# muzishen/RCDMs

Measured on AMD Instinct MI355X. Metric: story-frames/sec (stage-2 UNet, 50-step DDIM, 512^2), higher is better.
Workload: dtype f16; 1 GPU; PororoSV stage-2, 512x512, 50-step DDIM, CFG 2.0, batch=1 story x 5 frames per GPU, ctx 85x768, random-init 1276.9M-param UNet3D; stories_per_gpu=1, latent=64, ddim_steps=50, parallelism=story-replicas x1

## Files before the change

include/rcdm.h:

```cpp
#ifndef RCDM_H
#define RCDM_H

#include <stddef.h>
#include <stdint.h>

#ifdef __cplusplus
extern "C" {
#endif

#define RCDM_VERSION 0x000300

#define RCDM_OK 0
#define RCDM_EINVAL (-1)
#define RCDM_ESHAPE (-2)
#define RCDM_ELAUNCH (-3)
#define RCDM_EWORKSPACE (-4)
#define RCDM_ECOMM (-5)

#define RCDM_EPI_BIAS 1
#define RCDM_EPI_ROWVEC 2
#define RCDM_EPI_RESIDUAL 4
#define RCDM_EPI_GELU 16
#define RCDM_EPI_GEGLU 8
#define RCDM_EPI_QUICK_GELU 32
// ... 124 lines not shown
int rcdm_pack_conv3x3_wino(const float* w, int32_t c_out, int32_t c_in, void* dst, void* stream);
int rcdm_upsample_taps_gather(const void* P, int32_t ldp, int32_t n_img, int32_t h, int32_t w, int32_t c_out, const float* bias,
                              void* out, int32_t ldc, void* stream);
int rcdm_conv_taps_gather(const void* P, int32_t ldp, int32_t n_img, int32_t h, int32_t w, int32_t c_out, int32_t upsample,
                          const float* bias, void* out, int32_t ldc, void* stream);
int rcdm_set_wino_slab_f16(int32_t on);
int rcdm_conv3x3_wino(const rcdm_conv3x3_desc* d, const rcdm_groupnorm_desc* gn, const float* gn_stat,
                      const float* gn_gamma, const float* gn_beta, const void* in, const void* in2, const void* U,
                      const void* W2, const float* bias, const float* rowvec, const void* residual, void* out,
                      void* workspace, size_t workspace_bytes, const rcdm_groupnorm_desc* gn_out, float* gn_out_partial,
                      void* stream);

typedef struct {
  int32_t M, C, ldx, ldy;
  float eps;
  int32_t rows_per_frame, frames;
} rcdm_layernorm_desc;

int rcdm_layernorm(const rcdm_layernorm_desc* d, const void* x, const float* gamma,
                   const float* beta, const float* pe, void* y, void* stream);

#define RCDM_ATTN_WIDE_RANGE 1
typedef struct {
  int32_t batch, heads, Lq, Lk, d;
  int32_t ldq, ldk, ldv, ldo;
  float scale;
  int32_t flags;
} rcdm_attn_desc;

int rcdm_flash_attn(const rcdm_attn_desc* d, const void* Q, const void* K, const void* V, void* out,
                    void* stream);
int rcdm_flash_attn_masked(const rcdm_attn_desc* d, const void* Q, const void* K, const void* V,
                           const unsigned char* key_valid, int32_t causal, void* out, void* stream);

size_t rcdm_xattn_image_bytes(int32_t batch, int32_t heads, int32_t d);
int rcdm_xattn_pack_kv(const void* K, const void* V, int32_t batch, int32_t Lk, int32_t heads, int32_t d, int32_t ldk,
                       int32_t ldv, void* image, void* stream);
int rcdm_xattn(const rcdm_attn_desc* d, const void* Q, const void* image, void* out, void* stream);

typedef struct {
  int32_t samples, frames, pixels, heads, d;
  int32_t ldqkv, ldo;
  float scale;
} rcdm_temporal_attn_desc;

int rcdm_temporal_attn(const rcdm_temporal_attn_desc* d, const void* qkv, void* out, void* stream);

typedef struct {
  int32_t M, C;
  int32_t ldx, ldo;
  float eps;
} rcdm_ff_desc;
size_t rcdm_ff_stream_bytes(int32_t C);
int rcdm_ff_fused_supported(int32_t C);
int rcdm_pack_ff_stream(const float* w1, const float* b1, const float* w2, int32_t C, void* wstream, float* b1_packed,
                        void* stream);
int rcdm_ff_fused(const rcdm_ff_desc* d, const void* x, const float* ln_gamma, const float* ln_beta, const void* wstream,
                  const float* b1_packed, const float* b2, void* out, void* stream);

typedef struct {
  int32_t M, C;
  int32_t lda, ldr, ldt, ldo;
  int32_t tail;
  int32_t rows_per_frame, frames;
  float eps;
  int32_t gn_groups, gn_rows;
// ... 324 lines not shown
```

rcdms_amd/csrc/attn.hip:

```cpp
#include <stdlib.h>
#include "common.h"
#include "attn_wide.h"

long long* g_attn_trace = nullptr;

namespace {

constexpr int KT = 64;

struct AttnArgs {
  const f16* Q;
  const f16* K;
  const f16* V;
  f16* O;
  int batch, heads, Lq, Lk, d, dch;
  int ldq, ldk, ldv, ldo;
  float c;
  const unsigned char* kvalid;
  int causal;
  int plain_order;
  int wide;
  long long* trace;
};

// ... 10 lines not shown
  return r;
}

constexpr float MSUB_THR = 6.0f;

template <int DS, int QF, bool PIPE, bool MASKED, int NW, int MD = 0>
__global__ __launch_bounds__(NW * 64, (MASKED && DS >= 5) ? 1 : 2) void flash_attn_kernel(const AttnArgs p) {
  constexpr bool MSUB = MD > 0;
  static_assert(!MSUB || (PIPE && !MASKED && MD < 16 * DS), "MSUB: pipelined, unmasked kernel with a spare QK^T column only");
  constexpr int DF = (DS + 1) / 2;
  constexpr int KP = 16 * DS + 8;
  constexpr int NT = NW * 64;
  constexpr int NSLOT = (KT * 2 * DS + NT - 1) / NT;
  constexpr int BQ = NW * 32 * QF;
  constexpr int VR = v_row_halfs(DF);
  constexpr int SK = KT * KP, SV = KT * VR;
  extern __shared__ __attribute__((aligned(16))) char smem[];
  f16* sK = (f16*)smem;
  f16* sV = sK + 2 * SK;

  const int t = threadIdx.x, lane = t & 63, wave = t >> 6;
  const int lr = lane & 31, hi = lane >> 5;
  const int nqb = (p.Lq + BQ - 1) / BQ;
  int item;
  {
    const int total = nqb * p.heads * p.batch, lin = blockIdx.x;
    const int xcd = lin & 7, q = total >> 3, r = total & 7;
    item = (xcd < r ? xcd * (q + 1) : r * (q + 1) + (xcd - r) * q) + (lin >> 3);
    if (p.plain_order) item = lin;
  }
  const int qb = item % nqb, bh = item / nqb;
  const int h = bh % p.heads, b = bh / p.heads;
  const int q0 = qb * BQ + wave * 32 * QF + lr;
  const bool ones_row = (DS & 1) ? true : p.d < 32 * DF;

  for (int i = t; i < (2 * SK + 2 * SV) / 8; i += NT) ((uint4*)smem)[i] = make_uint4(0, 0, 0, 0);
  __syncthreads();
  if (ones_row && t < 2 * KT) sV[(t >> 6) * SV + (t & 63) * VR + p.d] = (f16)1.0f;
  if (MSUB && t < 2 * KT) sK[(t >> 6) * SK + (t & 63) * KP + p.d] = (f16)1.0f;
  constexpr int sd_frag = MD >> 4, sd_hi = (MD >> 3) & 1, sd_e = MD & 7;

  f16x8 qf[QF][DS];
#pragma unroll
  for (int j = 0; j < QF; ++j)
#pragma unroll
    for (int s = 0; s < DS; ++s) {
      const int dc = s * 16 + hi * 8;
      Pack16 v;
      v.u = make_uint4(0, 0, 0, 0);
      if (q0 + 32 * j < p.Lq && dc < p.d)
        v.u = *(const uint4*)(p.Q + ((size_t)b * p.Lq + q0 + 32 * j) * p.ldq + h * p.d + dc);
      if (MSUB) {
#pragma unroll
        for (int e = 0; e < 8; ++e) v.e[e] = (f16)((float)v.e[e] * p.c);
      }
      qf[j][s] = v.h;
    }
  float m_sub[QF], m_issue[QF];
#pragma unroll
  for (int j = 0; j < QF; ++j) m_sub[j] = m_issue[j] = 0.f;

  f32x16 oacc[QF][DF];
  float m_run[QF], l_run[QF];
#pragma unroll
  for (int j = 0; j < QF; ++j) {
    m_run[j] = -INFINITY;
// ... 220 lines not shown
    }

    RCDM_ATTN_STAMP(tr_sm);
#pragma unroll
    for (int f = 0; f < DF; ++f)
#pragma unroll
      for (int st = 0; st < 4; ++st) {
        const f16* vp = sV + par * SV + v_rd + (16 * st) * VR + 32 * f;
        union { s16x4 h[2]; f16x8 v; } vf;
        vf.h[0] = lds_read_tr16(vp);
        vf.h[1] = lds_read_tr16(vp + 8 * VR);
#pragma unroll
        for (int j = 0; j < QF; ++j) oacc[j][f] = __builtin_amdgcn_mfma_f32_32x32x16_f16(vf.v, pf[j][st], oacc[j][f], 0, 0, 0);
        if constexpr (DS == 10) __builtin_amdgcn_sched_barrier(0);
      }
    RCDM_ATTN_STAMP(tr_pv);
  };

  if constexpr (PIPE) {
    for (int kt = 0; kt < ntiles; kt += 2) {
      step(kt, s_even, s_odd);
      if (kt + 1 < ntiles) step(kt + 1, s_odd, s_even);
    }
  } else {
    for (int kt = 0; kt < ntiles; ++kt) step(kt, s_even, s_even);
  }
#ifdef RCDM_ATTN_TRACE
  if (p.trace && lane == 0) {
    long long* o = p.trace + ((size_t)blockIdx.x * NW + (threadIdx.x >> 6)) * 8;
    o[0] = __builtin_amdgcn_s_memtime() - tr_begin; o[1] = tr_sync; o[2] = tr_qk; o[3] = tr_sm; o[4] = tr_pv; o[5] = ntiles;
  }
#endif

#pragma unroll
  for (int j = 0; j < QF; ++j) {
    float l_tot;
    if (ones_row) {
      float l0 = 0.f;
#pragma unroll
      for (int f = 0; f < DF; ++f)
#pragma unroll
        for (int rr = 0; rr < 16; rr += 4)
          if (f * 32 + rr * 2 == p.d) l0 = oacc[j][f][rr];
      l_tot = __shfl(l0, lr, 64);
    } else {
      l_tot = l_run[j] + __shfl_xor(l_run[j], 32, 64);
    }
    const float inv = l_tot > 0.f ? 1.f / l_tot : 0.f;
    const int q = q0 + 32 * j;
    if (q < p.Lq) {
      f16* ob = p.O + ((size_t)b * p.Lq + q) * p.ldo + h * p.d;
#pragma unroll
      for (int f = 0; f < DF; ++f)
#pragma unroll
        for (int g = 0; g < 4; ++g) {
          const int dd = f * 32 + 8 * g + 4 * hi;
          if (dd < p.d) {
            f16x4 o = {(f16)(oacc[j][f][4 * g] * inv), (f16)(oacc[j][f][4 * g + 1] * inv),
                       (f16)(oacc[j][f][4 * g + 2] * inv), (f16)(oacc[j][f][4 * g + 3] * inv)};
            *(f16x4*)(ob + dd) = o;
          }
        }
    }
  }
}

int attn_xcd_mode() {
  static const int mode = rcdm_env_int("RCDM_ATTN_XCD", 1);
  return mode;
}

template <int DS>
int launch_flash(const AttnArgs& a_in, hipStream_t stream) {
  constexpr int DF = (DS + 1) / 2;
  constexpr int KP = 16 * DS + 8;
  const size_t lds = (size_t)2 * (KT * KP + KT * v_row_halfs(DF)) * sizeof(f16);
  const int xcd_mode = attn_xcd_mode();
  AttnArgs a = a_in;
  a.plain_order = xcd_mode ? 0 : 1;
  if (a.kvalid || a.causal) {
    dim3 grid(((a.Lq + 127) / 128) * a.heads * a.batch);
    hipLaunchKernelGGL((flash_attn_kernel<DS, 1, (DS <= 5), true, 4>), grid, dim3(256), lds, stream, a);
  } else {
    dim3 grid(((a.Lq + 127) / 128) * a.heads * a.batch);
    static const int msub_mode = rcdm_env_int("RCDM_ATTN_MSUB", 1);
    {
      if constexpr (DS == 3) {
        if (msub_mode && !a.wide && a.d == 40 && a.Lk >= 4 * KT) {
          hipLaunchKernelGGL((flash_attn_kernel<DS, 1, true, false, 4, 40>), grid, dim3(256), lds, stream, a);
          return rcdm_check_launch();
        }
      }
    }
    hipLaunchKernelGGL((flash_attn_kernel<DS, 1, (DS <= 5), false, 4>), grid, dim3(256), lds, stream, a);
  }
  return rcdm_check_launch();
}

struct XAttnArgs {
  const f16* Q;
  const f16* KF;
  const f16* VF;
  f16* O;
  int batch, heads, Lq, Lk, d;
  int ldq, ldo;
  float c;
  int qi;
};

template <int DS, int NW>
__global__ __launch_bounds__(NW * 64, (NW == 8 && DS <= 3) ? 4 : 2) void xattn_kernel(const XAttnArgs p) {
  constexpr int DF = (DS + 1) / 2;
  constexpr int NFRAG = 3 * DS + 6 * DF;
  extern __shared__ __attribute__((aligned(16))) char xa_smem[];
  const int lane = threadIdx.x & 63, wave = threadIdx.x >> 6;
  const int lr = lane & 31, hi = lane >> 5;
  constexpr int BQ = NW * 32;
  const int nqb = (p.Lq + BQ - 1) / BQ;
  constexpr bool PF = DS <= 3;
  const int qi = PF ? p.qi : 1;
  const int npb = (nqb + qi - 1) / qi;
  const int bh = blockIdx.x / npb, qb0 = (blockIdx.x - bh * npb) * qi;
  const int b = bh / p.heads, h = bh - b * p.heads;
  const bool ones_row = (DS & 1) ? true : p.d < 32 * DF;
  constexpr f32x16 zero = {0.f, 0.f, 0.f, 0.f, 0.f, 0.f, 0.f, 0.f, 0.f, 0.f, 0.f, 0.f, 0.f, 0.f, 0.f, 0.f};
  {
    const uint4* srck = (const uint4*)(p.KF + (size_t)bh * 3 * DS * 512);
    const uint4* srcv = (const uint4*)(p.VF + (size_t)bh * 6 * DF * 512);
// ... 124 lines not shown
  const int per_bh = (3 * DS + 6 * DF) * 64;
  if (idx >= (size_t)batch * heads * per_bh) return;
  const int bh = (int)(idx / per_bh), r = (int)(idx - (size_t)bh * per_bh);
  const int frag = r >> 6, lane = r & 63, lr = lane & 31, hi = lane >> 5;
  const int h = bh % heads, b = bh / heads;
  union { f16 e[8]; uint4 u; } o;
  if (frag < 3 * DS) {
    const int kt = frag / DS, s = frag - kt * DS;
    const int key = kt * 32 + lr, dc = s * 16 + hi * 8;
#pragma unroll
    for (int i = 0; i < 8; ++i)
      o.e[i] = (key < Lk && dc + i < d) ? K[((size_t)b * Lk + key) * ldk + h * d + dc + i] : (f16)0.f;
    *(uint4*)(img_k + ((size_t)bh * 3 * DS + frag) * 512 + lane * 8) = o.u;
  } else {
    const int fv = frag - 3 * DS, f = fv / 6, st = fv - f * 6;
    const int dd = f * 32 + lr;
    const bool ones = d < 32 * DF && dd == d;
#pragma unroll
    for (int i = 0; i < 8; ++i) {
      const int key = 16 * st + (i < 4 ? 4 * hi + i : 8 + 4 * hi + (i - 4));
      float v = ones ? 1.0f : 0.0f;
      if (dd < d && key < Lk) v = (float)V[((size_t)b * Lk + key) * ldv + h * d + dd];
      o.e[i] = (f16)v;
    }
    *(uint4*)(img_v + ((size_t)bh * 6 * DF + fv) * 512 + lane * 8) = o.u;
  }
}

struct TAttnArgs {
  const f16* qkv;
  f16* out;
  int samples, pixels, heads, d, ldqkv, ldo, tpb;
  int g;
  float scale;
};

template <int F>
__global__ __launch_bounds__(256) void temporal_attn_kernel(const TAttnArgs p) {
  extern __shared__ __attribute__((aligned(16))) char smem[];
  f16* tile = (f16*)smem;
  const int t = threadIdx.x;
  const int C = p.heads * p.d, C3 = 3 * C;
  const int rowc = C3 / 8;
  const long total_px = (long)p.samples * p.pixels;
  const long px0 = (long)blockIdx.x * p.tpb;

  const int lane = t & 63, wave = t >> 6;
  const int nrows = p.tpb * F;
  constexpr int SU = 4;
  for (int r0 = wave; r0 < nrows; r0 += 4 * SU) {
    const f16* src[SU];
    f16* dst[SU];
    bool ok[SU], live[SU];
#pragma unroll
    for (int u = 0; u < SU; ++u) {
      const int r = r0 + 4 * u;
      live[u] = r < nrows;
      const int f = r % F, pl = r / F;
      const int px = (int)px0 + pl;
      ok[u] = live[u] && px < (int)total_px;
      const int b = ok[u] ? px / p.pixels : 0, pix = px - b * p.pixels;
      src[u] = p.qkv + ((long)(b * F + f) * p.pixels + (ok[u] ? pix : 0)) * (long)p.ldqkv;
      dst[u] = tile + (size_t)(live[u] ? r : 0) * C3;
    }
    for (int c = lane; c < rowc; c += 64) {
      uint4 v[SU];
// ... 52 lines not shown
    for (int c = sub * 8; c < p.d; c += 8 * p.g) {
      float o[8];
#pragma unroll
      for (int e = 0; e < 8; ++e) o[e] = 0.f;
#pragma unroll
      for (int j = 0; j < F; ++j) {
        Pack16 vv;
        vv.u = *(const uint4*)(base + (size_t)j * C3 + 2 * C + c);
        const float pj = s[j] * inv;
#pragma unroll
        for (int e = 0; e < 8; ++e) o[e] = fmaf(pj, (float)vv.e[e], o[e]);
      }
      Pack16 ov;
#pragma unroll
      for (int e = 0; e < 8; ++e) ov.e[e] = (f16)o[e];
      *(uint4*)(qrow + c) = ov.u;
    }
  }
  __syncthreads();

  const int outc = C / 8;
  for (int r = wave; r < nrows; r += 4) {
    const int f = r % F, pl = r / F;
    const int px = (int)px0 + pl;
    if (px < (int)total_px) {
      const int b = px / p.pixels, pix = px - b * p.pixels;
      f16* dst = p.out + ((long)(b * F + f) * p.pixels + pix) * (long)p.ldo;
      const f16* srow = tile + (size_t)r * C3;
      for (int c = lane; c < outc; c += 64) *(uint4*)(dst + c * 8) = *(const uint4*)(srow + c * 8);
    }
  }
}

}

extern "C" {

int rcdm_flash_attn_masked(const rcdm_attn_desc* d, const void* Q, const void* K, const void* V,
                           const unsigned char* key_valid, int32_t causal, void* out, void* stream_) {
  if (!d || !Q || !K || !V || !out) return RCDM_EINVAL;
  if (d->batch <= 0 || d->heads <= 0 || d->Lq <= 0 || d->Lk <= 0 || d->d <= 0) return RCDM_EINVAL;
  const bool wide_head = d->d > 160;
  if (wide_head ? (d->d > 512 || (d->d & 63) || key_valid || causal) : (d->d & 7) != 0) return RCDM_ESHAPE;
  if ((d->ldq & 7) || (d->ldk & 7) || (d->ldv & 7) || (d->ldo & 3)) return RCDM_ESHAPE;
  if ((size_t)(d->Lk + 4 * 64) * (size_t)(d->ldk > d->ldv ? d->ldk : d->ldv) * 2 >= 0x7FFFFFFFull) return RCDM_ESHAPE;
  if (wide_head) {
    if ((size_t)d->Lq * (size_t)(d->ldq > d->ldo ? d->ldq : d->ldo) * 2 >= 0x7FFFFFFFull) return RCDM_ESHAPE;
    const int xcd_mode = attn_xcd_mode();
    AttnWideArgs w;
    w.Q = (const f16*)Q; w.K = (const f16*)K; w.V = (const f16*)V; w.O = (f16*)out;
    w.batch = d->batch; w.heads = d->heads; w.Lq = d->Lq; w.Lk = d->Lk; w.d = d->d;
    w.ldq = d->ldq; w.ldk = d->ldk; w.ldv = d->ldv; w.ldo = d->ldo;
    w.c = d->scale * 1.4426950408889634f;
    w.plain_order = xcd_mode ? 0 : 1;
    return rcdm_attn_wide_launch(w, (hipStream_t)stream_);
  }
  AttnArgs a;
  a.Q = (const f16*)Q; a.K = (const f16*)K; a.V = (const f16*)V; a.O = (f16*)out;
  a.batch = d->batch; a.heads = d->heads; a.Lq = d->Lq; a.Lk = d->Lk; a.d = d->d; a.dch = d->d / 8;
  a.ldq = d->ldq; a.ldk = d->ldk; a.ldv = d->ldv; a.ldo = d->ldo;
  a.c = d->scale * 1.4426950408889634f;
  a.kvalid = key_valid;
  a.wide = (d->flags & RCDM_ATTN_WIDE_RANGE) != 0;
  a.causal = causal ? 1 : 0;
  a.trace = g_attn_trace;
  hipStream_t stream = (hipStream_t)stream_;
  const int ds = (d->d + 15) / 16;
  if (ds <= 1) return launch_flash<1>(a, stream);
  if (ds <= 2) return launch_flash<2>(a, stream);
  if (ds <= 3) return launch_flash<3>(a, stream);
  if (ds <= 5) return launch_flash<5>(a, stream);
  static const int ds7_mode = rcdm_env_int("RCDM_ATTN_DS7", 1);
  if (ds7_mode && (ds == 6 || ds == 7)) return launch_flash<7>(a, stream);
  return launch_flash<10>(a, stream);
}

int rcdm_debug_set_attn_trace(void* device_buffer) {
  g_attn_trace = (long long*)device_buffer;
  return RCDM_OK;
}

int rcdm_flash_attn(const rcdm_attn_desc* d, const void* Q, const void* K, const void* V, void* out, void* stream_) {
  return rcdm_flash_attn_masked(d, Q, K, V, nullptr, 0, out, stream_);
}

static int xattn_ds(int d) {
  const int ds = (d + 15) / 16;
  return ds <= 3 ? ds : ds <= 5 ? 5 : 10;
}

size_t rcdm_xattn_image_bytes(int32_t batch, int32_t heads, int32_t d) {
  if (batch <= 0 || heads <= 0 || d <= 0 || (d & 7) || d > 160) return 0;
  const int DS = xattn_ds(d), DF = (DS + 1) / 2;
  return (size_t)batch * heads * (3 * DS + 6 * DF) * 1024;
}

int rcdm_xattn_pack_kv(const void* K, const void* V, int32_t batch, int32_t Lk, int32_t heads, int32_t d, int32_t ldk,
                       int32_t ldv, void* image, void* stream_) {
  if (!K || !V || !image || batch <= 0 || heads <= 0 || Lk <= 0 || d <= 0) return RCDM_EINVAL;
  if ((d & 7) || d > 160 || Lk > 96 || ldk < heads * d || ldv < heads * d) return RCDM_ESHAPE;
  const int DS = xattn_ds(d), DF = (DS + 1) / 2;
  const size_t total = (size_t)batch * heads * (3 * DS + 6 * DF) * 64;
  f16* img_k = (f16*)image;
  f16* img_v = img_k + (size_t)batch * heads * 3 * DS * 512;
  hipLaunchKernelGGL(xattn_pack_kv_kernel, dim3((unsigned)((total + 255) / 256)), dim3(256), 0, (hipStream_t)stream_,
                     (const f16*)K, (const f16*)V, batch, Lk, heads, d, ldk, ldv, DS, DF, img_k, img_v);
  return rcdm_check_launch();
// ... 34 lines not shown
    hipLaunchKernelGGL((xattn_kernel<DS_, 4>), grid, block, lds, stream, a);          \
  else                                                                                \
    hipLaunchKernelGGL((xattn_kernel<DS_, 8>), grid, block, lds, stream, a)
  switch (DS) {
    case 1: XA_LAUNCH(1); break;
    case 2: XA_LAUNCH(2); break;
    case 3: XA_LAUNCH(3); break;
    case 5: XA_LAUNCH(5); break;
    default: XA_LAUNCH(10); break;
  }
#undef XA_LAUNCH
  return rcdm_check_launch();
}

int rcdm_temporal_attn(const rcdm_temporal_attn_desc* d, const void* qkv, void* out, void* stream_) {
  if (!d || !qkv || !out) return RCDM_EINVAL;
  if (d->samples <= 0 || d->pixels <= 0 || d->heads <= 0 || d->d <= 0) return RCDM_EINVAL;
  if (d->frames < 1 || d->frames > 8 || (d->d & 7) || (d->ldqkv & 7) || (d->ldo & 7)) return RCDM_ESHAPE;
  TAttnArgs a;
  a.qkv = (const f16*)qkv; a.out = (f16*)out; a.samples = d->samples; a.pixels = d->pixels;
  a.heads = d->heads; a.d = d->d; a.ldqkv = d->ldqkv; a.ldo = d->ldo; a.scale = d->scale;
  const int C = d->heads * d->d;
  const size_t px_bytes = (size_t)d->frames * 3 * C * sizeof(f16);
  static const int lds_cap_kb = rcdm_env_int("RCDM_TATTN_KB", 32);
  int tpb = (int)(((size_t)lds_cap_kb * 1024) / px_bytes);
  const int by_threads = 256 / (d->heads * d->frames);
  if (tpb > by_threads) tpb = by_threads;
  if (tpb < 1) tpb = 1;
  if ((size_t)tpb * px_bytes > 160 * 1024 || d->heads * d->frames > 256) return RCDM_ESHAPE;
  a.tpb = tpb;
  int g = 8;
  while (g > 1 && (tpb * d->heads * d->frames * g > 256 || d->d / 8 < g)) g >>= 1;
  a.g = g;
  const size_t lds = (size_t)tpb * px_bytes;
  hipStream_t stream = (hipStream_t)stream_;
  const long total_px = (long)d->samples * d->pixels;
  dim3 grid((unsigned)((total_px + tpb - 1) / tpb)), block(256);
#define TA_LAUNCH(F)                                                                                              \
  {                                                                                                               \
    static size_t lds_set = 0;                                                                                    \
    if (lds > lds_set) {                                                                                          \
      (void)hipFuncSetAttribute((const void*)temporal_attn_kernel<F>, hipFuncAttributeMaxDynamicSharedMemorySize, \
                                (int)lds);                                                                        \
      lds_set = lds;                                                                                              \
    }                                                                                                             \
    hipLaunchKernelGGL(temporal_attn_kernel<F>, grid, block, lds, stream, a);                                     \
  }
  switch (d->frames) {
    case 1: TA_LAUNCH(1); break;
    case 2: TA_LAUNCH(2); break;
    case 3: TA_LAUNCH(3); break;
    case 4: TA_LAUNCH(4); break;
    case 5: TA_LAUNCH(5); break;
    case 6: TA_LAUNCH(6); break;
    case 7: TA_LAUNCH(7); break;
    default: TA_LAUNCH(8); break;
  }
#undef TA_LAUNCH
  return rcdm_check_launch();
}

}
```

rcdms_amd/hip.py:

```python
import ctypes as C
import os
import sys

import torch

_HERE = os.path.dirname(os.path.abspath(__file__))
LIB_PATH = os.environ.get("RCDM_LIB") or os.path.join(_HERE, "lib", "librcdm_hip.so")

EPI_BIAS, EPI_ROWVEC, EPI_RESIDUAL, EPI_GEGLU, EPI_GELU, EPI_QUICK_GELU, EPI_RELU = 1, 2, 4, 8, 16, 32, 64

_ERR = {-1: "RCDM_EINVAL", -2: "RCDM_ESHAPE", -3: "RCDM_ELAUNCH", -4: "RCDM_EWORKSPACE", -5: "RCDM_ECOMM"}


class RcdmError(RuntimeError):
    pass


class GemmDesc(C.Structure):
    _fields_ = [("M", C.c_int32), ("N", C.c_int32), ("K", C.c_int32),
                ("lda", C.c_int32), ("ldc", C.c_int32), ("ldr", C.c_int32),
                ("epilogue", C.c_int32), ("rows_per_sample", C.c_int32), ("ldt", C.c_int32),
                ("out_scale", C.c_float), ("split_k", C.c_int32), ("dup_rows", C.c_int32)]


# ... 172 lines not shown
    "rcdm_gemm_lnx_parts_ok": (C.c_int, [C.POINTER(GemmDesc), _I, _I]),
    "rcdm_gemm_plan_query": (C.c_int, [C.POINTER(GemmDesc), _I, _I, C.POINTER(C.c_int32)]),
    "rcdm_conv3x3_plan_query": (C.c_int, [C.POINTER(ConvDesc), C.POINTER(C.c_int32)]),
    "rcdm_gemm_lnx_workspace_bytes": (C.c_size_t, [C.POINTER(GemmDesc), _I, _I]),
    "rcdm_set_groupnorm_fold": (C.c_int, [_I]),
    "rcdm_gemm_lnx": (C.c_int, [C.POINTER(GemmDesc), C.POINTER(Lnx), _P, _P, _P, _P, _P, _P, _P, _SZ, _P]),
    "rcdm_gemm_workspace_bytes": (_SZ, [C.POINTER(GemmDesc)]),
    "rcdm_set_igemm_variant": (C.c_int, [_I]),
    "rcdm_set_shape_rules": (C.c_int, [C.c_char_p]),
    "rcdm_set_igemm_pingpong": (C.c_int, [_I]),
    "rcdm_debug_set_igemm_trace": (C.c_int, [_P]),
    "rcdm_debug_set_attn_trace": (C.c_int, [_P]),
    "rcdm_debug_mfma_peak": (C.c_int, [C.c_int32, C.c_int32, _P, _P, _P]),
    "rcdm_gemm": (C.c_int, [C.POINTER(GemmDesc), _P, _P, _P, _P, _P, _P, _P, _SZ, _P]),
    "rcdm_conv3x3_workspace_bytes": (_SZ, [C.POINTER(ConvDesc)]),
    "rcdm_conv3x3": (C.c_int, [C.POINTER(ConvDesc), _P, _P, _P, _P, _P, _P, _P, _SZ, _P]),
    "rcdm_conv3x3_add1x1": (C.c_int, [C.POINTER(ConvDesc), _P, _P, _P, _P, _P, _P, _P, _P, _SZ, _P]),
    "rcdm_conv3x3_add1x1_gnstat": (C.c_int, [C.POINTER(ConvDesc), C.POINTER(GroupNormDesc), _P, _P, _P, _P, _P, _P, _P, _P, _SZ, _P, _SZ, _P]),
    "rcdm_groupnorm_workspace_bytes": (_SZ, [C.POINTER(GroupNormDesc)]),
    "rcdm_groupnorm_silu": (C.c_int, [C.POINTER(GroupNormDesc), _P, _P, _P, _P, _P, _SZ, _P]),
    "rcdm_groupnorm_stats": (C.c_int, [C.POINTER(GroupNormDesc), _P, _P, _P, _SZ, _P]),
    "rcdm_groupnorm_stats_prestat": (C.c_int, [C.POINTER(GroupNormDesc), _P, _P, _SZ, _P]),
    "rcdm_groupnorm_prestat_ok": (C.c_int, [C.POINTER(GroupNormDesc)]),
    "rcdm_groupnorm_silu_prestat": (C.c_int, [C.POINTER(GroupNormDesc), _P, _P, _P, _P, _P, _SZ, _P]),
    "rcdm_gemm_gnstat_ok": (C.c_int, [C.POINTER(GemmDesc), C.POINTER(GroupNormDesc)]),
    "rcdm_gemm_gnstat": (C.c_int, [C.POINTER(GemmDesc), C.POINTER(GroupNormDesc), _P, _P, _P, _P, _P, _P, _P, _SZ, _P, _SZ, _P]),
    "rcdm_conv3x3_gnstat_ok": (C.c_int, [C.POINTER(ConvDesc), C.POINTER(GroupNormDesc)]),
    "rcdm_conv3x3_gnstat": (C.c_int, [C.POINTER(ConvDesc), C.POINTER(GroupNormDesc), _P, _P, _P, _P, _P, _P, _P, _SZ, _P, _SZ, _P]),
    "rcdm_softmax_rows": (C.c_int, [_I, _I, _I, _I, C.c_float, _P, _P, _P]),
    "rcdm_layernorm": (C.c_int, [C.POINTER(LayerNormDesc), _P, _P, _P, _P, _P, _P]),
    "rcdm_flash_attn": (C.c_int, [C.POINTER(AttnDesc), _P, _P, _P, _P, _P]),
    "rcdm_flash_attn_masked": (C.c_int, [C.POINTER(AttnDesc), _P, _P, _P, _P, _I, _P, _P]),
    "rcdm_temporal_attn": (C.c_int, [C.POINTER(TemporalAttnDesc), _P, _P, _P]),
    "rcdm_ff_stream_bytes": (_SZ, [_I]),
    "rcdm_ff_fused_supported": (C.c_int, [_I]),
    "rcdm_pack_ff_stream": (C.c_int, [_P, _P, _P, _I, _P, _P, _P]),
    "rcdm_ff_fused": (C.c_int, [C.POINTER(FFDesc), _P, _P, _P, _P, _P, _P, _P, _P]),
    "rcdm_rowchain_supported": (C.c_int, [_I]),
    "rcdm_rowchain_config_supported": (C.c_int, [_I, _I, _I]),
    "rcdm_rowchain_stream_bytes": (_SZ, [_I, _I]),
    "rcdm_pack_rowchain": (C.c_int, [_P, _I, _I, _P, _P, _P, _P, _P, _P, _P]),
    "rcdm_rowchain": (C.c_int, [C.POINTER(RowChainDesc), _P, _P, _P, _P, _P, _P, _P, _P, _P, _P, _P, _P, _P, _P, _P, _P, _P]),
    "rcdm_timestep_embed": (C.c_int, [_P, _I, _I, _P, _P]),
    "rcdm_small_linear": (C.c_int, [_P, _I, _I, _P, _P, _I, _I, _I, _P, _P]),
    "rcdm_assemble_input": (C.c_int, [_P, _P, _P, _I, _I, _I, _I, _I, _P, _I, _I, _P]),
    "rcdm_ncfhw_to_rows": (C.c_int, [_P, _I, _I, _I, _I, _I, _P, _I, _I, _P]),
    "rcdm_rows_to_ncfhw": (C.c_int, [_P, _I, _I, _I, _I, _I, _I, _P, _P]),
    "rcdm_cfg_ddim_step": (C.c_int, [_P, _I, _P, _I, _I, _I, _I, _I, _F, _P, _P, _P]),
    "rcdm_cfg_pndm_step": (C.c_int, [_P, _I, _P, _P, _I, _I, _I, _I, _I, _F, _P, _P, _P]),
    "rcdm_cfg_sigma_step": (C.c_int, [_P, _I, _P, _P, _P, _P, _I, _I, _I, _I, _I, _F, _P, _P, _P]),
    "rcdm_cfg_rescale_workspace_bytes": (_SZ, [_I, _I, _I, _I]),
    "rcdm_cfg_rescale_factor": (C.c_int, [_P, _I, _I, _I, _I, _I, _F, _F, _P, _SZ, _P, _P]),
    "rcdm_cfg_ddim_step_scaled": (C.c_int, [_P, _I, _P, _I, _I, _I, _I, _I, _F, _P, _P, _P, _P]),
    "rcdm_cfg_pndm_step_scaled": (C.c_int, [_P, _I, _P, _P, _I, _I, _I, _I, _I, _F, _P, _P, _P, _P]),
    "rcdm_cfg_sigma_step_scaled": (C.c_int, [_P, _I, _P, _P, _P, _P, _I, _I, _I, _I, _I, _F, _P, _P, _P, _P]),
    "rcdm_prior_assemble": (C.c_int, [_P, _P, _P, _I, _P, _P, _I, _I, _I, _I, _I, _P]),
    "rcdm_cfg_unclip_step": (C.c_int, [_P, _I, _P, _I, _I, _I, C.c_float, C.c_float, _P, _P, _P, _P]),
    "rcdm_embed_tokens": (C.c_int, [_P, _I, _I, _P, _I, _P, _I, _P, _I, _P]),
    "rcdm_patch_rows": (C.c_int, [_P, _I, _I, _I, _I, _P, _I, _P]),
    "rcdm_load_timestep": (C.c_int, [_P, _P, _P, _I, _P]),
    "rcdm_image_resample_lds_bytes": (_SZ, [C.POINTER(ResampleDesc)]),
    "rcdm_image_resample": (C.c_int, [C.POINTER(ResampleDesc), _P, _P, _P, _P, _P, _P, _P]),
    "rcdm_frames_to_u8": (C.c_int, [C.POINTER(FramesU8Desc), _P, _P, _P]),
    "rcdm_conv2d": (C.c_int, [C.POINTER(Conv2dDesc), _P, _P, _P, _P, _P]),
    "rcdm_pool2d": (C.c_int, [C.POINTER(Pool2dDesc), _P, _P, _P]),
    "rcdm_global_avgpool": (C.c_int, [_I, _I, _I, _P, C.c_int64, _P, C.c_int64, _P]),
# ... 230 lines not shown
    _check(load().rcdm_gemm_plan_query(C.byref(desc), int(bool(producer)), int(bool(consumer)), out), "rcdm_gemm_plan_query")
    return dict(zip(_PLAN_FIELDS, out))


def conv3x3_plan_query(desc):
    out = (C.c_int32 * 8)()
    _check(load().rcdm_conv3x3_plan_query(C.byref(desc), out), "rcdm_conv3x3_plan_query")
    return dict(zip(_PLAN_FIELDS, out))


def gemm_lnx_parts_ok(desc, parts, consumer=False):
    return bool(load().rcdm_gemm_lnx_parts_ok(C.byref(desc), int(parts), int(bool(consumer))))


def gemm_lnx_workspace_bytes(desc, producer=False, consumer=False):
    return int(load().rcdm_gemm_lnx_workspace_bytes(C.byref(desc), int(bool(producer)), int(bool(consumer))))


def gemm_lnx(desc, lnx, a, w, bias, rowvec, residual, out, workspace, workspace_bytes, stream=None):
    _check(load().rcdm_gemm_lnx(C.byref(desc), C.byref(lnx), a, w, bias, rowvec, residual, out, workspace, workspace_bytes,
                                stream_ptr() if stream is None else stream), "rcdm_gemm_lnx")


def flash_attn(desc, q, k, v, out, stream=None):
    _check(load().rcdm_flash_attn(C.byref(desc), q, k, v, out,
                                  stream_ptr() if stream is None else stream), "rcdm_flash_attn")


def flash_attn_masked(desc, q, k, v, key_valid, causal, out, stream=None):
    _check(load().rcdm_flash_attn_masked(C.byref(desc), q, k, v, key_valid, int(causal), out,
                                         stream_ptr() if stream is None else stream), "rcdm_flash_attn_masked")


def temporal_attn(desc, qkv, out, stream=None):
    _check(load().rcdm_temporal_attn(C.byref(desc), qkv, out,
                                     stream_ptr() if stream is None else stream), "rcdm_temporal_attn")


def ff_stream_bytes(Cc):
    return load().rcdm_ff_stream_bytes(Cc)


def ff_fused_supported(Cc):
    return bool(load().rcdm_ff_fused_supported(Cc))


def rowchain_supported(Cc):
    return bool(load().rcdm_rowchain_supported(Cc))


def rowchain_config_supported(Cc, tail, pe_frames=0):
    return bool(load().rcdm_rowchain_config_supported(Cc, tail, pe_frames))


def rowchain_stream_bytes(Cc, tail):
    return load().rcdm_rowchain_stream_bytes(Cc, tail)


def pack_rowchain(wa, Cc, tail, wt, w1, b1, w2, wstream, b1p, stream=None):
    _check(load().rcdm_pack_rowchain(wa, Cc, tail, wt, w1, b1, w2, wstream, b1p,
                                     stream_ptr() if stream is None else stream), "rcdm_pack_rowchain")


def rowchain(desc, a_in, res, tok, a_bias, ln_g, ln_b, pe, wstream, b1p, b2, out, stream=None, gn_stat=None, gn_g=None,
             gn_b=None, z_res=None, z_bias=None):
    _check(load().rcdm_rowchain(C.byref(desc), a_in, res, tok, a_bias, ln_g, ln_b, pe, wstream, b1p, b2, out,
# ... 468 lines not shown
```

Before: 6.267 story-frames/s.

## Split temporal attention heads across blocks and add 2-wave flash attention option

Adds a temporal attention kernel that assigns a group of heads per block instead of whole pixels, choosing heads-per-block so the grid has enough blocks for the CU count. It is enabled by default when one pixel occupies a block. It also adds an optional 2-wave flash attention variant for d=40/80 unmasked attention, selectable via env or API, plus a plan-query API. The split raises parallelism for small-pixel levels but reloads nothing extra, at the cost of more, smaller blocks.

```diff
diff --git a/include/rcdm.h b/include/rcdm.h
--- a/include/rcdm.h
+++ b/include/rcdm.h
@@ -180,6 +180,8 @@
                     void* stream);
 int rcdm_flash_attn_masked(const rcdm_attn_desc* d, const void* Q, const void* K, const void* V,
                            const unsigned char* key_valid, int32_t causal, void* out, void* stream);
+int rcdm_flash_attn_plan_query(const rcdm_attn_desc* d, int32_t masked, int32_t out[8]);
+int rcdm_set_attn_nw(int32_t nw);
 
 size_t rcdm_xattn_image_bytes(int32_t batch, int32_t heads, int32_t d);
 int rcdm_xattn_pack_kv(const void* K, const void* V, int32_t batch, int32_t Lk, int32_t heads, int32_t d, int32_t ldk,
diff --git a/rcdms_amd/csrc/attn.hip b/rcdms_amd/csrc/attn.hip
--- a/rcdms_amd/csrc/attn.hip
+++ b/rcdms_amd/csrc/attn.hip
@@ -66,6 +66,7 @@
   const int qb = item % nqb, bh = item / nqb;
   const int h = bh % p.heads, b = bh / p.heads;
   const int q0 = qb * BQ + wave * 32 * QF + lr;
+  const int wave_s = __builtin_amdgcn_readfirstlane(wave);
   const bool ones_row = (DS & 1) ? true : p.d < 32 * DF;
 
   for (int i = t; i < (2 * SK + 2 * SV) / 8; i += NT) ((uint4*)smem)[i] = make_uint4(0, 0, 0, 0);
@@ -352,6 +353,13 @@
   }
 #endif
 
+  int e_lr = lr, e_hi = hi, e_q0 = q0;
+  if constexpr (NW == 2) {
+    const int e_lane = __builtin_amdgcn_mbcnt_hi(~0u, __builtin_amdgcn_mbcnt_lo(~0u, 0u));
+    e_lr = e_lane & 31;
+    e_hi = e_lane >> 5;
+    e_q0 = qb * BQ + wave_s * 32 * QF + e_lr;
+  }
 #pragma unroll
   for (int j = 0; j < QF; ++j) {
     float l_tot;
@@ -362,19 +370,19 @@
 #pragma unroll
         for (int rr = 0; rr < 16; rr += 4)
           if (f * 32 + rr * 2 == p.d) l0 = oacc[j][f][rr];
-      l_tot = __shfl(l0, lr, 64);
+      l_tot = __shfl(l0, e_lr, 64);
     } else {
       l_tot = l_run[j] + __shfl_xor(l_run[j], 32, 64);
     }
     const float inv = l_tot > 0.f ? 1.f / l_tot : 0.f;
-    const int q = q0 + 32 * j;
+    const int q = e_q0 + 32 * j;
     if (q < p.Lq) {
       f16* ob = p.O + ((size_t)b * p.Lq + q) * p.ldo + h * p.d;
 #pragma unroll
       for (int f = 0; f < DF; ++f)
 #pragma unroll
         for (int g = 0; g < 4; ++g) {
-          const int dd = f * 32 + 8 * g + 4 * hi;
+          const int dd = f * 32 + 8 * g + 4 * e_hi;
           if (dd < p.d) {
             f16x4 o = {(f16)(oacc[j][f][4 * g] * inv), (f16)(oacc[j][f][4 * g + 1] * inv),
                        (f16)(oacc[j][f][4 * g + 2] * inv), (f16)(oacc[j][f][4 * g + 3] * inv)};
@@ -390,30 +398,53 @@
   return mode;
 }
 
+int g_attn_nw = -1;
+int attn_nw_mode() {
+  if (g_attn_nw < 0) g_attn_nw = rcdm_env_int("RCDM_ATTN_NW", 0) == 2 ? 2 : 4;
+  return g_attn_nw;
+}
+
 template <int DS>
-int launch_flash(const AttnArgs& a_in, hipStream_t stream) {
+int launch_flash(const AttnArgs& a_in, hipStream_t stream, int32_t* plan = nullptr) {
   constexpr int DF = (DS + 1) / 2;
   constexpr int KP = 16 * DS + 8;
   const size_t lds = (size_t)2 * (KT * KP + KT * v_row_halfs(DF)) * sizeof(f16);
   const int xcd_mode = attn_xcd_mode();
   AttnArgs a = a_in;
   a.plain_order = xcd_mode ? 0 : 1;
-  if (a.kvalid || a.causal) {
-    dim3 grid(((a.Lq + 127) / 128) * a.heads * a.batch);
+  const int blocks4 = ((a.Lq + 127) / 128) * a.heads * a.batch;
+  const dim3 grid(blocks4);
+  const bool masked = a.kvalid || a.causal;
+  static const int msub_mode = rcdm_env_int("RCDM_ATTN_MSUB", 1);
+  const bool msub = DS == 3 && !masked && msub_mode && !a.wide && a.d == 40 && a.Lk >= 4 * KT;
+  const bool has2 = !masked && (DS == 5 || msub);
+  const int nw = has2 ? attn_nw_mode() : 4;
+  const dim3 grid2(((a.Lq + 63) / 64) * a.heads * a.batch);
+  if (plan) {
+    plan[0] = nw; plan[1] = nw * 32; plan[2] = (int32_t)(nw == 2 ? grid2.x : grid.x); plan[3] = (int32_t)lds;
+    plan[4] = msub; plan[5] = DS; plan[6] = KT; plan[7] = masked;
+    return RCDM_OK;
+  }
+  if (masked) {
     hipLaunchKernelGGL((flash_attn_kernel<DS, 1, (DS <= 5), true, 4>), grid, dim3(256), lds, stream, a);
-  } else {
-    dim3 grid(((a.Lq + 127) / 128) * a.heads * a.batch);
-    static const int msub_mode = rcdm_env_int("RCDM_ATTN_MSUB", 1);
-    {
-      if constexpr (DS == 3) {
-        if (msub_mode && !a.wide && a.d == 40 && a.Lk >= 4 * KT) {
-          hipLaunchKernelGGL((flash_attn_kernel<DS, 1, true, false, 4, 40>), grid, dim3(256), lds, stream, a);
-          return rcdm_check_launch();
-        }
-      }
-    }
-    hipLaunchKernelGGL((flash_attn_kernel<DS, 1, (DS <= 5), false, 4>), grid, dim3(256), lds, stream, a);
-  }
+    return rcdm_check_launch();
+  }
+  if constexpr (DS == 3) {
+    if (msub) {
+      if (nw == 2)
+        hipLaunchKernelGGL((flash_attn_kernel<DS, 1, true, false, 2, 40>), grid2, dim3(128), lds, stream, a);
+      else
+        hipLaunchKernelGGL((flash_attn_kernel<DS, 1, true, false, 4, 40>), grid, dim3(256), lds, stream, a);
+      return rcdm_check_launch();
+    }
+  }
+  if constexpr (DS == 5) {
+    if (nw == 2) {
+      hipLaunchKernelGGL((flash_attn_kernel<DS, 1, true, false, 2>), grid2, dim3(128), lds, stream, a);
+      return rcdm_check_launch();
+    }
+  }
+  hipLaunchKernelGGL((flash_attn_kernel<DS, 1, (DS <= 5), false, 4>), grid, dim3(256), lds, stream, a);
   return rcdm_check_launch();
 }
 
@@ -604,6 +635,7 @@
   f16* out;
   int samples, pixels, heads, d, ldqkv, ldo, tpb;
   int g;
+  int hpb;
   float scale;
 };
 
@@ -722,13 +754,114 @@
   }
 }
 
+template <int F>
+__global__ __launch_bounds__(256) void temporal_attn_heads_kernel(const TAttnArgs p) {
+  extern __shared__ __attribute__((aligned(16))) char smem[];
+  f16* tile = (f16*)smem;
+  const int t = threadIdx.x;
+  const int C = p.heads * p.d;
+  const int W = p.hpb * p.d, wc = W / 8;
+  const int nhg = p.heads / p.hpb;
+  const int px = blockIdx.x / nhg, hg = blockIdx.x - px * nhg;
+  const int b = px / p.pixels, pix = px - b * p.pixels;
+  const int col0 = hg * W;
+
+  constexpr int SU = 6;
+  const int nch = F * 3 * wc;
+  for (int i0 = t; i0 < nch; i0 += 256 * SU) {
+    uint4 v[SU];
+#pragma unroll
+    for (int u = 0; u < SU; ++u) {
+      const int idx = i0 + 256 * u;
+      v[u] = make_uint4(0, 0, 0, 0);
+      if (idx < nch) {
+        const int rs = idx / wc, c = idx - rs * wc;
+        const int f = rs / 3, sl = rs - f * 3;
+        v[u] = *(const uint4*)(p.qkv + ((long)(b * F + f) * p.pixels + pix) * (long)p.ldqkv + sl * C + col0 + c * 8);
+      }
+    }
+#pragma unroll
+    for (int u = 0; u < SU; ++u) {
+      const int idx = i0 + 256 * u;
+      if (idx < nch) *(uint4*)(tile + (size_t)idx * 8) = v[u];
+    }
+  }
+  __syncthreads();
+
+  const int items = p.hpb * F;
+  const int sub = t % p.g, item = t / p.g;
+  if (item < items) {
+    const int i = item % F, hl = item / F;
+    f16* base = tile + hl * p.d;
+    const int W3 = 3 * W;
+    f16* qrow = base + (size_t)i * W3;
+    float s[F];
+#pragma unroll
+    for (int j = 0; j < F; ++j) s[j] = 0.f;
+    for (int c = sub * 8; c < p.d; c += 8 * p.g) {
+      Pack16 qv;
+      qv.u = *(const uint4*)(qrow + c);
+#pragma unroll
+      for (int j = 0; j < F; ++j) {
+        Pack16 kv;
+        kv.u = *(const uint4*)(base + (size_t)j * W3 + W + c);
+        float acc = s[j];
+#pragma unroll
+        for (int e = 0; e < 8; ++e) acc = fmaf((float)qv.e[e], (float)kv.e[e], acc);
+        s[j] = acc;
+      }
+    }
+    for (int off = 1; off < p.g; off <<= 1) {
+#pragma unroll
+      for (int j = 0; j < F; ++j) s[j] += __shfl_xor(s[j], off, 64);
+    }
+    float mx = s[0] * p.scale;
+#pragma unroll
+    for (int j = 0; j < F; ++j) {
+      s[j] *= p.scale;
+      mx = fmaxf(mx, s[j]);
+    }
+    float sum = 0.f;
+#pragma unroll
+    for (int j = 0; j < F; ++j) {
+      s[j] = __expf(s[j] - mx);
+      sum += s[j];
+    }
+    const float inv = __builtin_amdgcn_rcpf(sum);
+    for (int c = sub * 8; c < p.d; c += 8 * p.g) {
+      float o[8];
+#pragma unroll
+      for (int e = 0; e < 8; ++e) o[e] = 0.f;
+#pragma unroll
+      for (int j = 0; j < F; ++j) {
+        Pack16 vv;
+        vv.u = *(const uint4*)(base + (size_t)j * W3 + 2 * W + c);
+        const float pj = s[j] * inv;
+#pragma unroll
+        for (int e = 0; e < 8; ++e) o[e] = fmaf(pj, (float)vv.e[e], o[e]);
+      }
+      Pack16 ov;
+#pragma unroll
+      for (int e = 0; e < 8; ++e) ov.e[e] = (f16)o[e];
+      *(uint4*)(qrow + c) = ov.u;
+    }
+  }
+  __syncthreads();
+
+  for (int idx = t; idx < F * wc; idx += 256) {
+    const int f = idx / wc, c = idx - f * wc;
+    *(uint4*)(p.out + ((long)(b * F + f) * p.pixels + pix) * (long)p.ldo + col0 + c * 8) =
+        *(const uint4*)(tile + (size_t)f * 3 * W + c * 8);
+  }
+}
+
 }
 
 extern "C" {
 
-int rcdm_flash_attn_masked(const rcdm_attn_desc* d, const void* Q, const void* K, const void* V,
-                           const unsigned char* key_valid, int32_t causal, void* out, void* stream_) {
-  if (!d || !Q || !K || !V || !out) return RCDM_EINVAL;
+static int flash_attn_dispatch(const rcdm_attn_desc* d, const void* Q, const void* K, const void* V,
+                               const unsigned char* key_valid, int32_t causal, void* out, void* stream_, int32_t* plan) {
+  if (!d || (!plan && (!Q || !K || !V || !out))) return RCDM_EINVAL;
   if (d->batch <= 0 || d->heads <= 0 || d->Lq <= 0 || d->Lk <= 0 || d->d <= 0) return RCDM_EINVAL;
   const bool wide_head = d->d > 160;
   if (wide_head ? (d->d > 512 || (d->d & 63) || key_valid || causal) : (d->d & 7) != 0) return RCDM_ESHAPE;
@@ -743,6 +876,11 @@
     w.ldq = d->ldq; w.ldk = d->ldk; w.ldv = d->ldv; w.ldo = d->ldo;
     w.c = d->scale * 1.4426950408889634f;
     w.plain_order = xcd_mode ? 0 : 1;
+    if (plan) {
+      plan[0] = 4; plan[1] = 128; plan[2] = ((d->Lq + 127) / 128) * d->heads * d->batch; plan[3] = 0;
+      plan[4] = 0; plan[5] = 0; plan[6] = 0; plan[7] = 0;
+      return RCDM_OK;
+    }
     return rcdm_attn_wide_launch(w, (hipStream_t)stream_);
   }
   AttnArgs a;
@@ -756,13 +894,30 @@
   a.trace = g_attn_trace;
   hipStream_t stream = (hipStream_t)stream_;
   const int ds = (d->d + 15) / 16;
-  if (ds <= 1) return launch_flash<1>(a, stream);
-  if (ds <= 2) return launch_flash<2>(a, stream);
-  if (ds <= 3) return launch_flash<3>(a, stream);
-  if (ds <= 5) return launch_flash<5>(a, stream);
+  if (ds <= 1) return launch_flash<1>(a, stream, plan);
+  if (ds <= 2) return launch_flash<2>(a, stream, plan);
+  if (ds <= 3) return launch_flash<3>(a, stream, plan);
+  if (ds <= 5) return launch_flash<5>(a, stream, plan);
   static const int ds7_mode = rcdm_env_int("RCDM_ATTN_DS7", 1);
-  if (ds7_mode && (ds == 6 || ds == 7)) return launch_flash<7>(a, stream);
-  return launch_flash<10>(a, stream);
+  if (ds7_mode && (ds == 6 || ds == 7)) return launch_flash<7>(a, stream, plan);
+  return launch_flash<10>(a, stream, plan);
+}
+
+int rcdm_flash_attn_masked(const rcdm_attn_desc* d, const void* Q, const void* K, const void* V,
+                           const unsigned char* key_valid, int32_t causal, void* out, void* stream_) {
+  return flash_attn_dispatch(d, Q, K, V, key_valid, causal, out, stream_, nullptr);
+}
+
+int rcdm_flash_attn_plan_query(const rcdm_attn_desc* d, int32_t masked, int32_t out[8]) {
+  if (!out) return RCDM_EINVAL;
+  static const unsigned char some_mask = 1;
+  return flash_attn_dispatch(d, nullptr, nullptr, nullptr, masked ? &some_mask : nullptr, 0, nullptr, nullptr, out);
+}
+
+int rcdm_set_attn_nw(int32_t nw) {
+  if (nw != -1 && nw != 0 && nw != 2 && nw != 4) return RCDM_EINVAL;
+  g_attn_nw = nw == 0 ? 4 : nw;
+  return RCDM_OK;
 }
 
 int rcdm_debug_set_attn_trace(void* device_buffer) {
@@ -863,12 +1018,36 @@
   int g = 8;
   while (g > 1 && (tpb * d->heads * d->frames * g > 256 || d->d / 8 < g)) g >>= 1;
   a.g = g;
-  const size_t lds = (size_t)tpb * px_bytes;
+  size_t lds = (size_t)tpb * px_bytes;
   hipStream_t stream = (hipStream_t)stream_;
   const long total_px = (long)d->samples * d->pixels;
   dim3 grid((unsigned)((total_px + tpb - 1) / tpb)), block(256);
+  static const int split_mode = rcdm_env_int("RCDM_TATTN_SPLIT", 1);
+  static const int hpb_mode = rcdm_env_int("RCDM_TATTN_HPB", 0);
+  a.hpb = 0;
+  if (split_mode && tpb == 1 && total_px * d->heads < 0x7FFFFFFFl) {
+    int hpb = d->heads;
+    const long want = 4l * rcdm_num_cus();
+    while (hpb > 1 && total_px * (d->heads / hpb) < want) {
+      int nxt = hpb - 1;
+      while (d->heads % nxt) --nxt;
+      hpb = nxt;
+    }
+    if (hpb_mode > 0 && hpb_mode <= d->heads && d->heads % hpb_mode == 0) hpb = hpb_mode;
+    a.hpb = hpb;
+    lds = (size_t)d->frames * 3 * hpb * d->d * sizeof(f16);
+    grid = dim3((unsigned)(total_px * (d->heads / hpb)));
+  }
 #define TA_LAUNCH(F)                                                                                              \
-  {                                                                                                               \
+  if (a.hpb) {                                                                                                    \
+    static size_t lds_set_h = 0;                                                                                  \
+    if (lds > lds_set_h) {                                                                                        \
+      (void)hipFuncSetAttribute((const void*)temporal_attn_heads_kernel<F>,                                       \
+                                hipFuncAttributeMaxDynamicSharedMemorySize, (int)lds);                            \
+      lds_set_h = lds;                                                                                            \
+    }                                                                                                             \
+    hipLaunchKernelGGL(temporal_attn_heads_kernel<F>, grid, block, lds, stream, a);                               \
+  } else {                                                                                                        \
     static size_t lds_set = 0;                                                                                    \
     if (lds > lds_set) {                                                                                          \
       (void)hipFuncSetAttribute((const void*)temporal_attn_kernel<F>, hipFuncAttributeMaxDynamicSharedMemorySize, \
diff --git a/rcdms_amd/hip.py b/rcdms_amd/hip.py
--- a/rcdms_amd/hip.py
+++ b/rcdms_amd/hip.py
@@ -228,6 +228,8 @@
     "rcdm_flash_attn": (C.c_int, [C.POINTER(AttnDesc), _P, _P, _P, _P, _P]),
     "rcdm_flash_attn_masked": (C.c_int, [C.POINTER(AttnDesc), _P, _P, _P, _P, _I, _P, _P]),
     "rcdm_temporal_attn": (C.c_int, [C.POINTER(TemporalAttnDesc), _P, _P, _P]),
+    "rcdm_flash_attn_plan_query": (C.c_int, [C.POINTER(AttnDesc), _I, C.POINTER(C.c_int32)]),
+    "rcdm_set_attn_nw": (C.c_int, [_I]),
     "rcdm_ff_stream_bytes": (_SZ, [_I]),
     "rcdm_ff_fused_supported": (C.c_int, [_I]),
     "rcdm_pack_ff_stream": (C.c_int, [_P, _P, _P, _I, _P, _P, _P]),
@@ -524,6 +526,19 @@
                                          stream_ptr() if stream is None else stream), "rcdm_flash_attn_masked")
 
 
+_ATTN_PLAN_FIELDS = ("waves", "block_queries", "blocks", "lds_bytes", "msub", "ds", "key_tile", "masked")
+
+
+def flash_attn_plan_query(desc, masked=False):
+    out = (C.c_int32 * 8)()
+    _check(load().rcdm_flash_attn_plan_query(C.byref(desc), int(bool(masked)), out), "rcdm_flash_attn_plan_query")
+    return dict(zip(_ATTN_PLAN_FIELDS, out))
+
+
+def set_attn_nw(nw):
+    _check(load().rcdm_set_attn_nw(int(nw)), "rcdm_set_attn_nw")
+
+
 def temporal_attn(desc, qkv, out, stream=None):
     _check(load().rcdm_temporal_attn(C.byref(desc), qkv, out,
                                      stream_ptr() if stream is None else stream), "rcdm_temporal_attn")
```

Result: no change. 6.288 story-frames/s, median of 6 (+0.3%).
